# mihikamd/DP-GSAT

Hardware: AMD Instinct MI355X
Metric: million edges/s (attn+sample+aggregate fwd+bwd) (higher is better)
Workload: dtype f32

## Files before the change

dp_gsat_amd/csrc/common.h:

```cpp
#pragma once
#include <cstring>
#include <cstdint>
#include <cstdio>
#include <cstdarg>
#include <hip/hip_runtime.h>

#include "../../include/gsat_hip.h"

namespace gsat {

void set_error(const char* fmt, ...);
const char* get_error();

#define GSAT_CHECK_HIP(expr)                                                                  \
    do {                                                                                      \
        hipError_t _e = (expr);                                                               \
        if (_e != hipSuccess) {                                                               \
            gsat::set_error("%s:%d: %s -> %s", __FILE__, __LINE__, #expr, hipGetErrorString(_e)); \
            return GSAT_ERR_HIP;                                                              \
        }                                                                                     \
    } while (0)

#define GSAT_REQUIRE(cond, code, ...)                                                         \
    do {                                                                                      \
        if (!(cond)) {                                                                        \
            gsat::set_error(__VA_ARGS__);                                                     \
            return (code);                                                                    \
        }                                                                                     \
    } while (0)

#define GSAT_LAUNCH_CHECK() GSAT_CHECK_HIP(hipGetLastError())

static inline int64_t ceil_div(int64_t a, int64_t b) { return (a + b - 1) / b; }

hipError_t zero_async(void* p, size_t bytes, hipStream_t stream);
static inline size_t align_up(size_t a, size_t b) { return (a + b - 1) / b * b; }

struct Arena {
    char* base;
    size_t cap, off;
    Arena(void* p, size_t bytes) : base(static_cast<char*>(p)), cap(bytes), off(0) {}
    template <class T> T* take(size_t n) {
        size_t b = align_up(n * sizeof(T), 256);
        if (base == nullptr || off + b > cap) { off += b; return nullptr; }
        T* r = reinterpret_cast<T*>(base + off);
        off += b;
        return r;
    }
    bool ok() const { return base != nullptr && off <= cap; }
};

struct SlabJob { const float* ws; int nslab; size_t slab; int M, N; int64_t ldc; int accumulate; float* out; };
int gemm_f32(hipStream_t stream, bool a_t, bool b_t, int64_t M, int64_t N, int64_t K, const float* A, int64_t lda, const float* B,
             int64_t ldb, float* C, int64_t ldc, const float* bias, bool accumulate, float* ws, size_t ws_floats, bool allow_split = false,
             SlabJob* defer = nullptr);
int slab_reduce_jobs(hipStream_t stream, const SlabJob* jobs, int n);
size_t gemm_workspace_floats(int64_t M, int64_t N, int64_t K, bool reduce_rows);

int aggr_sum_fwd_impl(hipStream_t stream, const float* x, const float* self_rows, const float* att, const float* edge_emb,
                      const int32_t* rowptr, const int32_t* col, const int32_t* eid, int64_t N, int64_t E, int64_t H, float self_coef,
                      float* out, const int32_t* chunk_ptr, float* partial);

#ifdef __HIPCC__
constexpr int WAVE = 64;

template <int CTRL> __device__ __forceinline__ float dpp_add(float v) {
    const int t = __builtin_amdgcn_update_dpp(0, __builtin_bit_cast(int, v), CTRL, 0xF, 0xF, true);
    return v + __builtin_bit_cast(float, t);
}

template <int WIDTH> __device__ __forceinline__ float group_sum(float v) {
    if constexpr ((WIDTH & (WIDTH - 1)) == 0) {
        if constexpr (WIDTH >= 2) v = dpp_add<0xB1>(v);
        if constexpr (WIDTH >= 4) v = dpp_add<0x4E>(v);
        if constexpr (WIDTH >= 8) v = dpp_add<0x141>(v);
        if constexpr (WIDTH >= 16) v = dpp_add<0x140>(v);
        if constexpr (WIDTH >= 32) v += __builtin_bit_cast(float, __builtin_amdgcn_ds_swizzle(__builtin_bit_cast(int, v), 0x401F));
        if constexpr (WIDTH >= 64) v += __shfl_xor(v, 32, 64);
    } else {
        const int l = (int)(threadIdx.x & 63) % WIDTH;
#pragma unroll
        for (int o = 16; o > 0; o >>= 1) {
            const float t = __shfl_down(v, o, 64);
            if (l + o < WIDTH) v += t;
        }
    }
    return v;
}

template <int LPR, int BLOCK> struct LaneGroups {
    static constexpr int GPW = 64 / LPR, GPB = (BLOCK / 64) * GPW;
    int grp, lane;
    __device__ __forceinline__ LaneGroups() {
        const int wl = threadIdx.x & 63, sub = wl / LPR;
        lane = wl % LPR;
        grp = sub < GPW ? (int)(threadIdx.x >> 6) * GPW + sub : -1;
    }
};

__device__ __forceinline__ float4 ld4(const float* p) { return *reinterpret_cast<const float4*>(p); }
__device__ __forceinline__ void st4(float* p, float4 v) { *reinterpret_cast<float4*>(p) = v; }
__device__ __forceinline__ void st4_nt(float* p, float4 v) {
    typedef float v4f __attribute__((ext_vector_type(4)));
    v4f t = {v.x, v.y, v.z, v.w};
    __builtin_nontemporal_store(t, reinterpret_cast<v4f*>(p));
}
__device__ __forceinline__ float4 f4zero() { return make_float4(0.f, 0.f, 0.f, 0.f); }
__device__ __forceinline__ float4 f4fma(float a, float4 x, float4 acc) {
    acc.x = fmaf(a, x.x, acc.x); acc.y = fmaf(a, x.y, acc.y);
    acc.z = fmaf(a, x.z, acc.z); acc.w = fmaf(a, x.w, acc.w);
    return acc;
}
__device__ __forceinline__ float f4dot(float4 a, float4 b) {
    return fmaf(a.x, b.x, fmaf(a.y, b.y, fmaf(a.z, b.z, a.w * b.w)));
}

__device__ __forceinline__ uint4 philox4x32(uint64_t seed, uint32_t c0, uint32_t c1, uint32_t c2, uint32_t c3) {
    uint32_t k0 = (uint32_t)seed, k1 = (uint32_t)(seed >> 32);
#pragma unroll
    for (int r = 0; r < 10; ++r) {
        uint64_t p0 = (uint64_t)0xD2511F53u * c0;
        uint64_t p1 = (uint64_t)0xCD9E8D57u * c2;
        uint32_t n0 = (uint32_t)(p1 >> 32) ^ c1 ^ k0;
        uint32_t n1 = (uint32_t)p1;
        uint32_t n2 = (uint32_t)(p0 >> 32) ^ c3 ^ k1;
        uint32_t n3 = (uint32_t)p0;
        c0 = n0; c1 = n1; c2 = n2; c3 = n3;
        k0 += 0x9E3779B9u; k1 += 0xBB67AE85u;
    }
    return make_uint4(c0, c1, c2, c3);
}

__device__ __forceinline__ float philox_noise_u(uint64_t seed, int row) {
    const uint4 r = philox4x32(seed, (uint32_t)row, 0u, 4u, 0x5A17u);
    return ((float)(r.x >> 9) + 0.5f) * (1.0f / 8388608.0f);
}

struct SeedRef {
    uint64_t value;
    const uint64_t* dev;
    __device__ __forceinline__ uint64_t get() const { return dev ? *dev : value; }
};

__device__ __forceinline__ float4 philox_keep4(uint64_t seed, int layer, int row, int c, float p) {
    uint4 r = philox4x32(seed, (uint32_t)row, (uint32_t)(c >> 2), (uint32_t)layer, 0x5A17u);
    const float k = 1.0f / 16777216.0f;
    return make_float4((float)(r.x >> 8) * k >= p ? 1.f : 0.f, (float)(r.y >> 8) * k >= p ? 1.f : 0.f,
                       (float)(r.z >> 8) * k >= p ? 1.f : 0.f, (float)(r.w >> 8) * k >= p ? 1.f : 0.f);
}
#endif

}
```

dp_gsat_amd/csrc/pna.hip:

```cpp
#include "common.h"
#include "pna_math.h"

namespace gsat {

constexpr int PNA_BLOCK = 128;
constexpr int SC_AMP = GSAT_SCALE_AMPLIFICATION, SC_ATT = GSAT_SCALE_ATTENUATION, SC_LIN = GSAT_SCALE_LINEAR, SC_INVLIN = GSAT_SCALE_INVERSE_LINEAR;

struct PnaCfg {
    int A, S;
    int aggr[8];
    int scal[8];
    float avg_lin, avg_log;
};

__device__ __forceinline__ int pna_xcd_remap(int b, int nb) {
    int q = nb >> 3, r = nb & 7, x = b & 7, i = b >> 3;
    return (x < r ? x * (q + 1) : r * (q + 1) + (x - r) * q) + i;
}

__device__ __forceinline__ float scaler_factor(int s, float deg, float avg_lin, float avg_log) {
    switch (s) {
        case SC_AMP: return logf(deg + 1.f) / avg_log;
        case SC_ATT: return deg == 0.f ? 1.f : avg_log / logf(deg + 1.f);
        case SC_LIN: return deg / avg_lin;
// ... 473 lines not shown
                P = make_float4(p0.x - mean.x * Q.x, p0.y - mean.y * Q.y, p0.z - mean.z * Q.z, p0.w - mean.w * Q.w);   \
            }
            GSAT_FOLD(ai, 0, Pi, Qi, gmn_i, gmx_i)
            {
#define GSAT_SELF(C)                                                                                                   \
            {                                                                                                          \
                const float xc = xi.C;                                                                                 \
                const float wlo = xc > 0.f ? amin : (xc < 0.f ? amax : wfirst), whi = xc > 0.f ? amax : (xc < 0.f ? amin : wfirst); \
                dxi.C = Pi.C * sa + Qi.C * xc * sa2 + gmn_i.C * wlo + gmx_i.C * whi;                                   \
                t1 = fmaf(Pi.C, xc, t1);                                                                               \
                t2 = fmaf(Qi.C * xc, xc, t2);                                                                          \
                tmn += xc > 0.f ? gmn_i.C * xc : (xc < 0.f ? gmx_i.C * xc : 0.f);                                      \
                tmx += xc > 0.f ? gmx_i.C * xc : (xc < 0.f ? gmn_i.C * xc : 0.f);                                      \
            }
            float4 dxi;
            GSAT_SELF(x) GSAT_SELF(y) GSAT_SELF(z) GSAT_SELF(w)
#undef GSAT_SELF
            st4(dx_self + (size_t)row * H + c, dxi);
            }
            GSAT_FOLD(aj, 1, Pj, Qj, gmn_j, gmx_j)
            if (HAS_EE) { GSAT_FOLD(ae, 2, Pe, Qe, gmn_e, gmx_e) }
#undef GSAT_FOLD
        }
        if (LONG) {
            float* r = partial + (size_t)chunk_ptr[row] * rec;
            if (on) {
                st4(r + c, Pj); st4(r + H + c, Qj); st4(r + 2 * H + c, gmn_j); st4(r + 3 * H + c, gmx_j);
                st4i(r + 4 * H + c, jmin); st4i(r + 5 * H + c, jmax);
                if (HAS_EE) {
                    float* re = r + 6 * H;
                    st4(re + c, Pe); st4(re + H + c, Qe); st4(re + 2 * H + c, gmn_e); st4(re + 3 * H + c, gmx_e);
                    st4i(re + 4 * H + c, emin); st4i(re + 5 * H + c, emax);
                }
            }
            const float s1 = group_sum<LPR>(t1), s2 = group_sum<LPR>(t2), smn = group_sum<LPR>(tmn), smx = group_sum<LPR>(tmx);
            if (lane == 0) {
                st4(r + (size_t)6 * GP * H, make_float4(s1, s2, smn, smx));
                st4(r + (size_t)6 * GP * H + 4, make_float4(__int_as_float(kmin_a), __int_as_float(kmax_a), 0.f, 0.f));
            }
            continue;
        }
        for (int kb = beg; kb < end; kb += 4) {
            const int nb = min(4, end - kb);
            int j4[4], e4[4];
            float w4[4];
            float4 x4[4], ee4[4];
            if (end - beg <= 4) {
#pragma unroll
                for (int u = 0; u < 4; ++u) { j4[u] = lj[u]; e4[u] = le[u]; w4[u] = lw[u]; }
            } else {
#pragma unroll
                for (int u = 0; u < 4; ++u) {
                    j4[u] = u < nb ? col[kb + u] : 0;
                    e4[u] = u < nb ? eid[kb + u] : 0;
                }
#pragma unroll
                for (int u = 0; u < 4; ++u) w4[u] = (u < nb && att) ? att[e4[u]] : 1.f;
            }
#pragma unroll
            for (int u = 0; u < 4; ++u) {
                x4[u] = (u < nb && on) ? ld4(x + (size_t)j4[u] * H + c) : f4zero();
                if (HAS_EE) ee4[u] = (u < nb && on) ? ld4(edge_emb + (size_t)e4[u] * H + c) : f4zero();
            }
#pragma unroll
            for (int u = 0; u < 4; ++u) {
                if (u >= nb) continue;
                const int k = kb + u, e = e4[u];
                const float w = w4[u];
                const float4 xj = x4[u];
                float da = 0.f;
                if (on) {
                    float4 dm;
                    dm.x = fmaf(Qj.x, w * xj.x, Pj.x) + (k == jmin.x ? gmn_j.x : 0.f) + (k == jmax.x ? gmx_j.x : 0.f);
                    dm.y = fmaf(Qj.y, w * xj.y, Pj.y) + (k == jmin.y ? gmn_j.y : 0.f) + (k == jmax.y ? gmx_j.y : 0.f);
                    dm.z = fmaf(Qj.z, w * xj.z, Pj.z) + (k == jmin.z ? gmn_j.z : 0.f) + (k == jmax.z ? gmx_j.z : 0.f);
                    dm.w = fmaf(Qj.w, w * xj.w, Pj.w) + (k == jmin.w ? gmn_j.w : 0.f) + (k == jmax.w ? gmx_j.w : 0.f);
                    st4(dmsg + (size_t)k * H + c, f4scale(w, dm));
                    da += f4dot(dm, xj);
                    da += t1 + w * t2 + (k == kmin_a ? tmn : 0.f) + (k == kmax_a ? tmx : 0.f);
                    if (HAS_EE) {
                        const float4 ee = ee4[u];
                        float4 de;
                        de.x = fmaf(Qe.x, w * ee.x, Pe.x) + (k == emin.x ? gmn_e.x : 0.f) + (k == emax.x ? gmx_e.x : 0.f);
                        de.y = fmaf(Qe.y, w * ee.y, Pe.y) + (k == emin.y ? gmn_e.y : 0.f) + (k == emax.y ? gmx_e.y : 0.f);
                        de.z = fmaf(Qe.z, w * ee.z, Pe.z) + (k == emin.z ? gmn_e.z : 0.f) + (k == emax.z ? gmx_e.z : 0.f);
                        de.w = fmaf(Qe.w, w * ee.w, Pe.w) + (k == emin.w ? gmn_e.w : 0.f) + (k == emax.w ? gmx_e.w : 0.f);
                        if (dedge) st4(dedge + (size_t)e * H + c, f4scale(w, de));
                        da += f4dot(de, ee);
                    }
                }
                if (datt) {
                    da = group_sum<LPR>(da);
                    if (lane == 0) datt[e] = c0 ? datt[e] + da : da;
                }
            }
        }
    }
}

constexpr int TILE_BLOCK = 512;

__global__ void k_pna_tiles(const int32_t* __restrict__ node_ptr, const int32_t* __restrict__ node_seg, const int32_t* __restrict__ rowptr,
                            const int32_t* __restrict__ rowptr_src, int N, int TN, int slack, int T, int4* __restrict__ desc,
                            int32_t* __restrict__ spill_count) {
    const int t = blockIdx.x * blockDim.x + threadIdx.x;
    if (t == 0 && spill_count) *spill_count = 0;
    if (t > T) return;
    const int64_t p = (int64_t)t * TN;
    int start = N;
    if (t < T && p < N) {
        start = (int)p;
        if (node_seg) {
            const int g0 = node_ptr[node_seg[p]];
            start = min((int)p, max(g0, (int)p - slack));
        }
    }
    desc[t] = make_int4(start, rowptr[start], rowptr_src[start], 0);
}

template <int LPR, int NAGG, bool NATT>
__global__ __launch_bounds__(TILE_BLOCK, 4) void k_pna_bwd_tile(
    const float* __restrict__ x, const float* __restrict__ att, const float* __restrict__ dout, const int32_t* __restrict__ rowptr,
    const int32_t* __restrict__ col, const int32_t* __restrict__ eid, const int4* __restrict__ desc,
    const int32_t* __restrict__ rowptr_src, const int32_t* __restrict__ slot_map, int H, int TE, int RCAP, float* dx,
    float* __restrict__ dmsg, float* datt, float* __restrict__ dw, const float* __restrict__ dx_add, int datt_acc) {
    constexpr int GPB = LaneGroups<LPR, TILE_BLOCK>::GPB;
    constexpr int RPW = 64 / LPR;
    constexpr int NSEG = NAGG * 2;
    extern __shared__ float4 smem4[];
    float4* erow = smem4;
    int* s_col = reinterpret_cast<int*>(erow + (size_t)TE * LPR);
    int* s_eid = s_col + TE;
    float* s_w = reinterpret_cast<float*>(s_eid);
    float* s_att = reinterpret_cast<float*>(s_eid + TE);
    int* s_slot = reinterpret_cast<int*>(s_att + TE);
    int* s_rp = s_slot + TE;
    int* s_rps = s_rp + RCAP + 1;
    float* s_na = reinterpret_cast<float*>(s_rps + RCAP + 1);
    float* s_dna = s_na + RCAP + 1;
    const int tid = threadIdx.x, wave = tid >> 6;
    const LaneGroups<LPR, TILE_BLOCK> lg;
    const int grp = lg.grp < 0 ? GPB : lg.grp;
    const int lane = lg.lane, c = lane * 4;
    const bool on = c < H && lg.grp >= 0;
    const int t = pna_xcd_remap(blockIdx.x, gridDim.x);
    const int4 d0 = desc[t], d1 = desc[t + 1];
    const int n0 = d0.x, n1 = d1.x;
    if (n1 <= n0) return;
    const int nr = n1 - n0;
    const int k0 = d0.y, ne = min(d1.y - k0, TE);
    const int s0 = d0.z, ns = d1.z - s0, nsl = min(ns, TE);
    float4 dcur[NSEG];
    float4 xi_cur = f4zero();
    const size_t out_stride = (size_t)NSEG * H;
    int row = lg.grp >= 0 ? n0 + grp : n1;
#pragma unroll
    for (int sg = 0; sg < NSEG; ++sg) dcur[sg] = f4zero();
    if (row < n1 && on) {
        const float* g0 = dout + (size_t)row * out_stride + c;
#pragma unroll
        for (int sg = 0; sg < NSEG; ++sg) dcur[sg] = ld4(g0 + (size_t)sg * H);
        xi_cur = ld4(x + (size_t)row * H + c);
    }
    for (int i = tid; i <= nr; i += TILE_BLOCK) {
        s_rp[i] = rowptr[n0 + i] - k0;
        s_rps[i] = rowptr_src[n0 + i] - s0;
        if (NATT) { s_na[i] = att[min(n0 + i, n1 - 1)]; s_dna[i] = 0.f; }
    }
    for (int i = tid; i < ne; i += TILE_BLOCK) {
        s_col[i] = col[k0 + i];
        if (!NATT) s_eid[i] = eid[k0 + i];
    }
    for (int i = tid; i < nsl; i += TILE_BLOCK) s_slot[i] = slot_map[s0 + i] - k0;
    __syncthreads();
    for (int base = 0; base < ne; base += GPB) {
        const int i = base + grp;
        if (i < ne && on)
            __builtin_amdgcn_global_load_lds((const __attribute__((address_space(1))) void*)(x + (size_t)s_col[i] * H + c),
                                             (__attribute__((address_space(3))) void*)(erow + (size_t)(base + wave * RPW) * LPR), 16, 0, 0);
    }
    for (int i = tid; i < ne; i += TILE_BLOCK) {
        if (NATT) {
            int lo = 0, hi = nr;
            while (hi - lo > 1) { const int mid = (lo + hi) >> 1; if (s_rp[mid] <= i) lo = mid; else hi = mid; }
            const float a = att[s_col[i]];
            s_att[i] = a;
            s_w[i] = a * s_na[lo];
        } else {
            s_att[i] = att ? att[s_eid[i]] : 1.f;
        }
    }
    asm volatile("s_waitcnt vmcnt(0)" ::: "memory");
    __syncthreads();
    for (; row < n1; row += GPB) {
        const int nrow = row + GPB;
        const int beg = s_rp[row - n0], end = s_rp[row - n0 + 1];
        const float cnt = (float)(end - beg);
        float sa = 0.f, sa2 = 0.f, amin = INFINITY, amax = -INFINITY;
        int kmin_a = beg, kmax_a = beg;
        Acc4 aj;
        aj.init();
        int4 jmin = make_int4(beg, beg, beg, beg), jmax = jmin;
        float wfirst = 1.f;
        for (int k = beg; k < end; ++k) {
            float w;
            float4 xv;
            if (k < ne) {
                w = NATT ? s_w[k] : s_att[k];
                xv = on ? erow[(size_t)k * LPR + lane] : f4zero();
            } else {
                w = NATT ? att[col[k0 + k]] * s_na[row - n0] : (att ? att[eid[k0 + k]] : 1.f);
                xv = on ? ld4(x + (size_t)col[k0 + k] * H + c) : f4zero();
            }
            if (k == beg) wfirst = w;
            sa += w; sa2 = fmaf(w, w, sa2);
            if (w < amin) { amin = w; kmin_a = k; }
            if (w > amax) { amax = w; kmax_a = k; }
            const float4 m = f4scale(w, xv);
            if (m.x < aj.mn.x) jmin.x = k; if (m.y < aj.mn.y) jmin.y = k; if (m.z < aj.mn.z) jmin.z = k; if (m.w < aj.mn.w) jmin.w = k;
            if (m.x > aj.mx.x) jmax.x = k; if (m.y > aj.mx.y) jmax.y = k; if (m.z > aj.mx.z) jmax.z = k; if (m.w > aj.mx.w) jmax.w = k;
            aj.add(m);
        }
        const float4 xi = xi_cur;
        const Acc4 ai = self_stats(xi, sa, sa2, amin, amax);
        const float n = fmaxf(cnt, 1.f), inv_n = 1.f / n;
        float t1 = 0.f, t2 = 0.f, tmn = 0.f, tmx = 0.f;
        float4 Pi, Qi, Pj, Qj, gmn_i, gmx_i, gmn_j, gmx_j;
#define GSAT_TFOLD(ACC, PART, P, Q, GMN, GMX)                                                                              \
        {                                                                                                                  \
            const float4 mean = f4scale(inv_n, ACC.s);                                                                     \
            const float4 var = make_float4(ACC.q.x * inv_n - mean.x * mean.x, ACC.q.y * inv_n - mean.y * mean.y,           \
                                           ACC.q.z * inv_n - mean.z * mean.z, ACC.q.w * inv_n - mean.w * mean.w);          \
            const float4 hs = make_float4(var.x > 0.f ? 0.5f * __builtin_amdgcn_rsqf(var.x + 1e-5f) : 0.f,                 \
                                          var.y > 0.f ? 0.5f * __builtin_amdgcn_rsqf(var.y + 1e-5f) : 0.f,                 \
                                          var.z > 0.f ? 0.5f * __builtin_amdgcn_rsqf(var.z + 1e-5f) : 0.f,                 \
                                          var.w > 0.f ? 0.5f * __builtin_amdgcn_rsqf(var.w + 1e-5f) : 0.f);                \
            float4 p0 = f4scale(inv_n, dcur[0 * 2 + (PART)]);                                                              \
            if (NAGG == 5) { const float4 vsum = dcur[(NAGG == 5 ? 4 : 0) * 2 + (PART)];                                   \
                             p0 = make_float4(p0.x + vsum.x, p0.y + vsum.y, p0.z + vsum.z, p0.w + vsum.w); }               \
            GMN = dcur[1 * 2 + (PART)];                                                                                    \
            GMX = dcur[2 * 2 + (PART)];                                                                                    \
            const float4 vs = dcur[3 * 2 + (PART)];                                                                        \
            const float4 gv = make_float4(vs.x * hs.x, vs.y * hs.y, vs.z * hs.z, vs.w * hs.w);                             \
            Q = f4scale(2.f * inv_n, gv);                                                                                  \
            P = make_float4(p0.x - mean.x * Q.x, p0.y - mean.y * Q.y, p0.z - mean.z * Q.z, p0.w - mean.w * Q.w);           \
        }
        GSAT_TFOLD(ai, 0, Pi, Qi, gmn_i, gmx_i)
        GSAT_TFOLD(aj, 1, Pj, Qj, gmn_j, gmx_j)
#undef GSAT_TFOLD
        if (nrow < n1 && on) {
            const float* g0 = dout + (size_t)nrow * out_stride + c;
#pragma unroll
            for (int sg = 0; sg < NSEG; ++sg) dcur[sg] = ld4(g0 + (size_t)sg * H);
            xi_cur = ld4(x + (size_t)nrow * H + c);
        }
        if (on) {
            float4 dxi;
#define GSAT_TSELF(C)                                                                                                      \
            {                                                                                                              \
                const float xc = xi.C;                                                                                     \
                const float wlo = xc > 0.f ? amin : (xc < 0.f ? amax : wfirst), whi = xc > 0.f ? amax : (xc < 0.f ? amin : wfirst); \
                dxi.C = Pi.C * sa + Qi.C * xc * sa2 + gmn_i.C * wlo + gmx_i.C * whi;                                       \
                t1 = fmaf(Pi.C, xc, t1);                                                                                   \
                t2 = fmaf(Qi.C * xc, xc, t2);                                                                              \
                tmn += xc > 0.f ? gmn_i.C * xc : (xc < 0.f ? gmx_i.C * xc : 0.f);                                          \
                tmx += xc > 0.f ? gmx_i.C * xc : (xc < 0.f ? gmn_i.C * xc : 0.f);                                          \
            }
            GSAT_TSELF(x) GSAT_TSELF(y) GSAT_TSELF(z) GSAT_TSELF(w)
#undef GSAT_TSELF
            if (end == beg) dxi = f4zero();
            st4(dx + (size_t)row * H + c, dxi);
        }
        for (int k = beg; k < end; ++k) {
            float w;
            float4 xj;
            int e = 0, j;
            if (k < ne) {
                w = NATT ? s_w[k] : s_att[k]; j = s_col[k];
                if (!NATT) e = s_eid[k];
                xj = on ? erow[(size_t)k * LPR + lane] : f4zero();
            } else {
                j = col[k0 + k];
                if (!NATT) e = eid[k0 + k];
                w = NATT ? att[j] * s_na[row - n0] : (att ? att[e] : 1.f);
                xj = on ? ld4(x + (size_t)j * H + c) : f4zero();
            }
            const bool in_lds = k < ne && j >= n0 && j < n1;
            float da = 0.f;
            if (on) {
                float4 dm;
                dm.x = fmaf(Qj.x, w * xj.x, Pj.x) + (k == jmin.x ? gmn_j.x : 0.f) + (k == jmax.x ? gmx_j.x : 0.f);
                dm.y = fmaf(Qj.y, w * xj.y, Pj.y) + (k == jmin.y ? gmn_j.y : 0.f) + (k == jmax.y ? gmx_j.y : 0.f);
                dm.z = fmaf(Qj.z, w * xj.z, Pj.z) + (k == jmin.z ? gmn_j.z : 0.f) + (k == jmax.z ? gmx_j.z : 0.f);
                dm.w = fmaf(Qj.w, w * xj.w, Pj.w) + (k == jmin.w ? gmn_j.w : 0.f) + (k == jmax.w ? gmx_j.w : 0.f);
                const float4 o = f4scale(w, dm);
                if (in_lds) erow[(size_t)k * LPR + lane] = o; else st4(dmsg + (size_t)(k0 + k) * H + c, o);
                da = f4dot(dm, xj) + t1 + w * t2 + (k == kmin_a ? tmn : 0.f) + (k == kmax_a ? tmx : 0.f);
            }
            if (datt) {
                da = group_sum<LPR>(da);
                if (NATT) {
                    if (lane == 0) {
                        s_dna[row - n0] = fmaf(da, k < ne ? s_att[k] : att[j], s_dna[row - n0]);
                        const float share = da * s_na[row - n0];
                        if (in_lds) s_w[k] = share; else dw[k0 + k] = share;
                    }
                } else if (lane == 0) datt[e] = da;
            }
        }
    }
    __syncthreads();
    for (int j = lg.grp >= 0 ? n0 + grp : n1; j < n1; j += GPB) {
        if (!on) continue;
        const int sb = s_rps[j - n0], se = s_rps[j - n0 + 1];
        float4 acc = ld4(dx + (size_t)j * H + c);
        const float dprev = (NATT && datt && datt_acc && lane == 0) ? datt[j] : 0.f;
        if (dx_add) {
            const float4 r = ld4(dx_add + (size_t)j * H + c);
            acc.x += r.x; acc.y += r.y; acc.z += r.z; acc.w += r.w;
        }
        float sw = 0.f;
        for (int s_ = sb; s_ < se; ++s_) {
            const int kl = s_ < nsl ? s_slot[s_] : slot_map[s0 + s_] - k0;
            if (kl >= 0 && kl < ne) {
                const float4 v = erow[(size_t)kl * LPR + lane];
                acc.x += v.x; acc.y += v.y; acc.z += v.z; acc.w += v.w;
                if (NATT) sw += s_w[kl];
            }
        }
        st4(dx + (size_t)j * H + c, acc);
        if (NATT && datt && lane == 0) datt[j] = (s_dna[j - n0] + sw) + dprev;
    }
}

__global__ void k_pna_spill_rows(const int4* __restrict__ desc, int TN, int TE, const int32_t* __restrict__ rowptr_src,
                                 const int32_t* __restrict__ slot_map, int num_rows, int32_t* __restrict__ spill_rows,
                                 int32_t* __restrict__ spill_count) {
    const int j = blockIdx.x * blockDim.x + threadIdx.x;
    if (j >= num_rows) return;
    const int sb = rowptr_src[j], se = rowptr_src[j + 1];
    if (sb == se) return;
    int t = j / TN;
    if (j >= desc[t + 1].x) ++t;
    const int k0 = desc[t].y, ne = min(desc[t + 1].y - k0, TE);
    bool flag = false;
    for (int s_ = sb; s_ < se && !flag; ++s_) {
        const int k = slot_map[s_];
        flag = k < k0 || k >= k0 + ne;
    }
    if (flag) {
        const int idx = atomicAdd(spill_count, 1);
        if (idx < num_rows) spill_rows[idx] = j;
    }
}

template <int LPR>
__global__ __launch_bounds__(256) void k_pna_bwd_spill(const float* __restrict__ dmsg, const int4* __restrict__ desc, int TN, int TE,
                                                       const int32_t* __restrict__ rowptr_src, const int32_t* __restrict__ slot_map,
                                                       const int32_t* __restrict__ spill_rows, const int32_t* __restrict__ spill_count,
                                                       int num_rows, int H, float* __restrict__ dx, const float* __restrict__ dw,
                                                       float* __restrict__ dna) {
    const LaneGroups<LPR, 256> lg;
    constexpr int GPB = LaneGroups<LPR, 256>::GPB;
    const int lane = lg.lane, c = lane * 4;
    const int count = min(*spill_count, num_rows);
    if (lg.grp < 0) return;
    for (int i = blockIdx.x * GPB + lg.grp; i < count; i += gridDim.x * GPB) {
        const int j = spill_rows[i];
        const int sb = rowptr_src[j], se = rowptr_src[j + 1];
        int t = j / TN;
        if (j >= desc[t + 1].x) ++t;
        const int k0 = desc[t].y, ne = min(desc[t + 1].y - k0, TE);
        if (c >= H) continue;
        float4 acc = ld4(dx + (size_t)j * H + c);
        float sw = 0.f;
        for (int s_ = sb; s_ < se; ++s_) {
            const int k = slot_map[s_];
            if (k >= k0 && k < k0 + ne) continue;
            const float4 v = ld4(dmsg + (size_t)k * H + c);
            acc.x += v.x; acc.y += v.y; acc.z += v.z; acc.w += v.w;
            if (dna) sw += dw[k];
        }
        st4(dx + (size_t)j * H + c, acc);
        if (dna && lane == 0) dna[j] += sw;
    }
}

static inline int pna_lpr(int64_t H) {
    if (H <= 0 || H % 4 != 0 || H > 256) return 0;
    int64_t q = H / 4;
    return q <= 4 ? 4 : q <= 8 ? 8 : q <= 16 ? 16 : q <= 20 ? 20 : q <= 32 ? 32 : 64;
}

constexpr int PNA_CHUNK = 256;
static inline bool pna_width_ok(int64_t H) { return H > 0 && H % 4 == 0 && H <= 512; }

static inline void pna_grid(int64_t N, int lpr, int* nb, int* rpg) {
    const int gpb = (PNA_BLOCK / 64) * (64 / lpr);
    int64_t b = ceil_div(N, gpb);
    if (b > 256 * 64) b = 256 * 64;
    if (b < 1) b = 1;
    *nb = (int)b;
    *rpg = (int)std::max<int64_t>(1, ceil_div(N, b * gpb));
}

static inline int fixed_aggregators(const PnaCfg& cfg) {
    if (cfg.S != 1 || cfg.scal[0] != 0 || (cfg.A != 4 && cfg.A != 5)) return 0;
    if (cfg.aggr[0] != AGG_MEAN || cfg.aggr[1] != AGG_MIN || cfg.aggr[2] != AGG_MAX || cfg.aggr[3] != GSAT_AGG_STD) return 0;
    if (cfg.A == 5 && cfg.aggr[4] != AGG_SUM) return 0;
    return cfg.A;
}

static int make_cfg(const int32_t* aggr, int A, const int32_t* scal, int S, float avg_lin, float avg_log, PnaCfg* cfg) {
    GSAT_REQUIRE(aggr && scal && A >= 1 && A <= 8 && S >= 1 && S <= 8, GSAT_ERR_ARG, "pna: need 1..8 aggregators and scalers");
    cfg->A = A; cfg->S = S; cfg->avg_lin = avg_lin; cfg->avg_log = avg_log;
    for (int i = 0; i < 8; ++i) { cfg->aggr[i] = 0; cfg->scal[i] = 0; }
    for (int i = 0; i < A; ++i) {
        GSAT_REQUIRE(aggr[i] >= 0 && aggr[i] <= 5, GSAT_ERR_ARG, "pna: unknown aggregator code %d", aggr[i]);
        cfg->aggr[i] = aggr[i];
    }
    for (int i = 0; i < S; ++i) {
        GSAT_REQUIRE(scal[i] >= 0 && scal[i] <= 4, GSAT_ERR_ARG, "pna: unknown scaler code %d", scal[i]);
        cfg->scal[i] = scal[i];
    }
    return GSAT_OK;
}

template <int L, int NA, bool NATT>
static hipError_t pna_tile_allow_lds(size_t lds) {
    static size_t allowed = 0;
    if (lds <= allowed) return hipSuccess;
    hipError_t e = hipFuncSetAttribute((const void*)k_pna_bwd_tile<L, NA, NATT>, hipFuncAttributeMaxDynamicSharedMemorySize, (int)lds);
    if (e == hipSuccess) allowed = lds;
    return e;
}

static size_t pna_tile_lds_bytes(int lpr, int edges_cap, int rows_cap) {
    return (size_t)edges_cap * ((size_t)lpr * 16 + 16) + (size_t)(rows_cap + 1) * 16;
}

}

using namespace gsat;

#define GSAT_LPR_DISPATCH(lpr, CALL) \
    switch (lpr) { case 4: CALL(4); break; case 8: CALL(8); break; case 16: CALL(16); break; case 20: CALL(20); break; case 32: CALL(32); break; default: CALL(64); break; }

extern "C" {

static int pna_fwd_impl(const char* who, const float* x, const float* att, const float* edge_emb, const int32_t* rowptr, const int32_t* col,
                        const int32_t* eid, int64_t N, int64_t E, int64_t H, const int32_t* aggregators, int A, const int32_t* scalers, int S,
                        float avg_deg_lin, float avg_deg_log, float* out, const int32_t* chunk_ptr, float* partial, hipStream_t stream,
                        float* scal_out = nullptr) {
    GSAT_REQUIRE(N >= 0 && N < (1ll << 31), GSAT_ERR_ARG, "%s: bad N", who);
    PnaCfg cfg;
    int rc = make_cfg(aggregators, A, scalers, S, avg_deg_lin, avg_deg_log, &cfg);
    if (rc) return rc;
    if (N == 0) return GSAT_OK;
    GSAT_REQUIRE(pna_width_ok(H), GSAT_ERR_UNSUPPORTED, "%s: H=%lld must be a multiple of 4 and <= 512", who, (long long)H);
    GSAT_REQUIRE(x && rowptr && out, GSAT_ERR_ARG, "%s: null pointer", who);
    GSAT_REQUIRE(chunk_ptr == nullptr || partial != nullptr, GSAT_ERR_ARG, "%s: chunk_ptr needs the record workspace", who);
    if (E <= CH) chunk_ptr = nullptr;
    const int nagg = fixed_aggregators(cfg);
    GSAT_REQUIRE(!scal_out || (nagg && !edge_emb && !chunk_ptr), GSAT_ERR_UNSUPPORTED,
                 "%s: the compact output needs (mean,min,max,std[,sum]) with the identity scaler, no edge features, no hub chunks", who);
    for (int c0 = 0; c0 < (int)H; c0 += PNA_CHUNK) {
        const int Hc = std::min<int>(PNA_CHUNK, (int)H - c0);
        const int lpr = pna_lpr(Hc);
        int nb, rpg;
        pna_grid(N, lpr, &nb, &rpg);
        const int gpb = (PNA_BLOCK / 64) * (64 / lpr);
        const int cb = chunk_ptr ? (int)std::min<int64_t>(ceil_div(pna_max_chunks(E), gpb), 256 * 16) : 0;
#define GO(L, EE, NA)                                                                                                                       \
    do {                                                                                                                                    \
        k_pna_fwd<L, EE, NA, false><<<nb, PNA_BLOCK, 0, stream>>>(x, att, edge_emb, rowptr, col, eid, (int)N, (int)H, cfg, out, rpg, c0, Hc, chunk_ptr, partial, scal_out); \
        if (cb) k_pna_fwd<L, EE, NA, true><<<cb, PNA_BLOCK, 0, stream>>>(x, att, edge_emb, rowptr, col, eid, (int)N, (int)H, cfg, out, rpg, c0, Hc, chunk_ptr, partial, scal_out); \
    } while (0)
#define CALL(L)                                                                                                              \
    do {                                                                                                                     \
        if (edge_emb) {                                                                                                      \
            if (cb) k_pna_chunk_stats<L, true><<<cb, PNA_BLOCK, 0, stream>>>(x, att, edge_emb, rowptr, col, eid, (int)N, (int)H, chunk_ptr, partial, c0, Hc); \
            if (nagg == 4) GO(L, true, 4); else if (nagg == 5) GO(L, true, 5); else GO(L, true, 0);                          \
        } else {                                                                                                             \
            if (cb) k_pna_chunk_stats<L, false><<<cb, PNA_BLOCK, 0, stream>>>(x, att, edge_emb, rowptr, col, eid, (int)N, (int)H, chunk_ptr, partial, c0, Hc); \
// ... 213 lines not shown
```

Measured before the change: 125.4.

## Streamline PNA tiled backward: window-relative 32-bit addressing, split LDS/global edge loops

Rewrites the tiled PNA backward kernel to address global data through per-tile base pointers with 32-bit byte offsets. It splits each row's edge loop into an LDS-resident part and a global part so the inner loops no longer branch per edge. The per-edge binary search that built s_w at tile setup is removed, and the weight is computed as att*na_row inline. Each row's d-node-attention is accumulated in a register, explicit LDS store intrinsics are used, and the last row's dx is kept in a register instead of being re-read from global memory. The aim is fewer address computations, branches and memory round-trips, at the cost of more code and a risk of 32-bit offset overflow on large tiles.

```diff
diff --git a/dp_gsat_amd/csrc/common.h b/dp_gsat_amd/csrc/common.h
--- a/dp_gsat_amd/csrc/common.h
+++ b/dp_gsat_amd/csrc/common.h
@@ -105,6 +105,18 @@
     v4f t = {v.x, v.y, v.z, v.w};
     __builtin_nontemporal_store(t, reinterpret_cast<v4f*>(p));
 }
+__device__ __forceinline__ float4 ld4_off(const float* base, uint32_t byte_off) {
+    return *reinterpret_cast<const float4*>(reinterpret_cast<const char*>(base) + byte_off);
+}
+__device__ __forceinline__ void st4_off(float* base, uint32_t byte_off, float4 v) {
+    *reinterpret_cast<float4*>(reinterpret_cast<char*>(base) + byte_off) = v;
+}
+__device__ __forceinline__ void st4_lds(float4* p, float4 v) {
+    typedef float v4f __attribute__((ext_vector_type(4)));
+    v4f t = {v.x, v.y, v.z, v.w};
+    *(__attribute__((address_space(3))) v4f*)p = t;
+}
+__device__ __forceinline__ void st1_lds(float* p, float v) { *(__attribute__((address_space(3))) float*)p = v; }
 __device__ __forceinline__ float4 f4zero() { return make_float4(0.f, 0.f, 0.f, 0.f); }
 __device__ __forceinline__ float4 f4fma(float a, float4 x, float4 acc) {
     acc.x = fmaf(a, x.x, acc.x); acc.y = fmaf(a, x.y, acc.y);
diff --git a/dp_gsat_amd/csrc/pna.hip b/dp_gsat_amd/csrc/pna.hip
--- a/dp_gsat_amd/csrc/pna.hip
+++ b/dp_gsat_amd/csrc/pna.hip
@@ -649,15 +649,18 @@
     const int s0 = d0.z, ns = d1.z - s0, nsl = min(ns, TE);
     float4 dcur[NSEG];
     float4 xi_cur = f4zero();
-    const size_t out_stride = (size_t)NSEG * H;
-    int row = lg.grp >= 0 ? n0 + grp : n1;
+    const uint32_t hb = (uint32_t)H * 4u, gb = NSEG * hb, cb = (uint32_t)c * 4u;
+    const float* gwin = dout + (size_t)n0 * NSEG * H;
+    const float* xwin = x + (size_t)n0 * H;
+    float* dxwin = dx + (size_t)n0 * H;
+    float* mwin = dmsg + (size_t)k0 * H;
+    int r = lg.grp >= 0 ? grp : nr;
 #pragma unroll
     for (int sg = 0; sg < NSEG; ++sg) dcur[sg] = f4zero();
-    if (row < n1 && on) {
-        const float* g0 = dout + (size_t)row * out_stride + c;
-#pragma unroll
-        for (int sg = 0; sg < NSEG; ++sg) dcur[sg] = ld4(g0 + (size_t)sg * H);
-        xi_cur = ld4(x + (size_t)row * H + c);
+    if (r < nr && on) {
+#pragma unroll
+        for (int sg = 0; sg < NSEG; ++sg) dcur[sg] = ld4_off(gwin, r * gb + sg * hb + cb);
+        xi_cur = ld4_off(xwin, r * hb + cb);
     }
     for (int i = tid; i <= nr; i += TILE_BLOCK) {
         s_rp[i] = rowptr[n0 + i] - k0;
@@ -678,20 +681,18 @@
     }
     for (int i = tid; i < ne; i += TILE_BLOCK) {
         if (NATT) {
-            int lo = 0, hi = nr;
-            while (hi - lo > 1) { const int mid = (lo + hi) >> 1; if (s_rp[mid] <= i) lo = mid; else hi = mid; }
-            const float a = att[s_col[i]];
-            s_att[i] = a;
-            s_w[i] = a * s_na[lo];
+            s_att[i] = att[s_col[i]];
         } else {
             s_att[i] = att ? att[s_eid[i]] : 1.f;
         }
     }
     asm volatile("s_waitcnt vmcnt(0)" ::: "memory");
     __syncthreads();
-    for (; row < n1; row += GPB) {
-        const int nrow = row + GPB;
-        const int beg = s_rp[row - n0], end = s_rp[row - n0 + 1];
+    float4 dx_keep = f4zero();
+    for (; r < nr; r += GPB) {
+        const int nr_ = r + GPB;
+        const int beg = s_rp[r], end = s_rp[r + 1];
+        const float na_row = NATT ? s_na[r] : 0.f;
         const float cnt = (float)(end - beg);
         float sa = 0.f, sa2 = 0.f, amin = INFINITY, amax = -INFINITY;
         int kmin_a = beg, kmax_a = beg;
@@ -699,25 +700,25 @@
         aj.init();
         int4 jmin = make_int4(beg, beg, beg, beg), jmax = jmin;
         float wfirst = 1.f;
-        for (int k = beg; k < end; ++k) {
-            float w;
-            float4 xv;
-            if (k < ne) {
-                w = NATT ? s_w[k] : s_att[k];
-                xv = on ? erow[(size_t)k * LPR + lane] : f4zero();
-            } else {
-                w = NATT ? att[col[k0 + k]] * s_na[row - n0] : (att ? att[eid[k0 + k]] : 1.f);
-                xv = on ? ld4(x + (size_t)col[k0 + k] * H + c) : f4zero();
-            }
+        const int mid = min(end, max(beg, ne));
+        auto stats = [&](int k, float w, float4 xv) {
             if (k == beg) wfirst = w;
             sa += w; sa2 = fmaf(w, w, sa2);
             if (w < amin) { amin = w; kmin_a = k; }
             if (w > amax) { amax = w; kmax_a = k; }
             const float4 m = f4scale(w, xv);
-            if (m.x < aj.mn.x) jmin.x = k; if (m.y < aj.mn.y) jmin.y = k; if (m.z < aj.mn.z) jmin.z = k; if (m.w < aj.mn.w) jmin.w = k;
-            if (m.x > aj.mx.x) jmax.x = k; if (m.y > aj.mx.y) jmax.y = k; if (m.z > aj.mx.z) jmax.z = k; if (m.w > aj.mx.w) jmax.w = k;
-            aj.add(m);
-        }
+#define GSAT_TARG(C)                                                                                                       \
+            if (m.C < aj.mn.C) { jmin.C = k; aj.mn.C = m.C; }                                                              \
+            if (m.C > aj.mx.C) { jmax.C = k; aj.mx.C = m.C; }
+            GSAT_TARG(x) GSAT_TARG(y) GSAT_TARG(z) GSAT_TARG(w)
+#undef GSAT_TARG
+            aj.s.x += m.x; aj.s.y += m.y; aj.s.z += m.z; aj.s.w += m.w;
+            aj.q.x = fmaf(m.x, m.x, aj.q.x); aj.q.y = fmaf(m.y, m.y, aj.q.y); aj.q.z = fmaf(m.z, m.z, aj.q.z); aj.q.w = fmaf(m.w, m.w, aj.q.w);
+        };
+        for (int k = beg; k < mid; ++k)
+            stats(k, NATT ? s_att[k] * na_row : s_att[k], on ? erow[(size_t)k * LPR + lane] : f4zero());
+        for (int k = mid; k < end; ++k)
+            stats(k, NATT ? att[col[k0 + k]] * na_row : (att ? att[eid[k0 + k]] : 1.f), on ? ld4(x + (size_t)col[k0 + k] * H + c) : f4zero());
         const float4 xi = xi_cur;
         const Acc4 ai = self_stats(xi, sa, sa2, amin, amax);
         const float n = fmaxf(cnt, 1.f), inv_n = 1.f / n;
@@ -743,14 +744,6 @@
             P = make_float4(p0.x - mean.x * Q.x, p0.y - mean.y * Q.y, p0.z - mean.z * Q.z, p0.w - mean.w * Q.w);           \
         }
         GSAT_TFOLD(ai, 0, Pi, Qi, gmn_i, gmx_i)
-        GSAT_TFOLD(aj, 1, Pj, Qj, gmn_j, gmx_j)
-#undef GSAT_TFOLD
-        if (nrow < n1 && on) {
-            const float* g0 = dout + (size_t)nrow * out_stride + c;
-#pragma unroll
-            for (int sg = 0; sg < NSEG; ++sg) dcur[sg] = ld4(g0 + (size_t)sg * H);
-            xi_cur = ld4(x + (size_t)nrow * H + c);
-        }
         if (on) {
             float4 dxi;
 #define GSAT_TSELF(C)                                                                                                      \
@@ -766,23 +759,18 @@
             GSAT_TSELF(x) GSAT_TSELF(y) GSAT_TSELF(z) GSAT_TSELF(w)
 #undef GSAT_TSELF
             if (end == beg) dxi = f4zero();
-            st4(dx + (size_t)row * H + c, dxi);
-        }
-        for (int k = beg; k < end; ++k) {
-            float w;
-            float4 xj;
-            int e = 0, j;
-            if (k < ne) {
-                w = NATT ? s_w[k] : s_att[k]; j = s_col[k];
-                if (!NATT) e = s_eid[k];
-                xj = on ? erow[(size_t)k * LPR + lane] : f4zero();
-            } else {
-                j = col[k0 + k];
-                if (!NATT) e = eid[k0 + k];
-                w = NATT ? att[j] * s_na[row - n0] : (att ? att[e] : 1.f);
-                xj = on ? ld4(x + (size_t)j * H + c) : f4zero();
-            }
-            const bool in_lds = k < ne && j >= n0 && j < n1;
+            if (nr_ < nr) st4_off(dxwin, r * hb + cb, dxi); else dx_keep = dxi;
+        }
+        GSAT_TFOLD(aj, 1, Pj, Qj, gmn_j, gmx_j)
+#undef GSAT_TFOLD
+        if (nr_ < nr && on) {
+#pragma unroll
+            for (int sg = 0; sg < NSEG; ++sg) dcur[sg] = ld4_off(gwin, nr_ * gb + sg * hb + cb);
+            xi_cur = ld4_off(xwin, nr_ * hb + cb);
+        }
+        float dna_acc = 0.f;
+        auto grad = [&](int k, float w, float a_src, int j, int e, float4 xj, bool lds) {
+            const bool in_lds = lds && j >= n0 && j < n1;
             float da = 0.f;
             if (on) {
                 float4 dm;
@@ -791,30 +779,43 @@
                 dm.z = fmaf(Qj.z, w * xj.z, Pj.z) + (k == jmin.z ? gmn_j.z : 0.f) + (k == jmax.z ? gmx_j.z : 0.f);
                 dm.w = fmaf(Qj.w, w * xj.w, Pj.w) + (k == jmin.w ? gmn_j.w : 0.f) + (k == jmax.w ? gmx_j.w : 0.f);
                 const float4 o = f4scale(w, dm);
-                if (in_lds) erow[(size_t)k * LPR + lane] = o; else st4(dmsg + (size_t)(k0 + k) * H + c, o);
+                if (in_lds) st4_lds(erow + (size_t)k * LPR + lane, o);
+                else if (lds) st4_off(mwin, k * hb + cb, o);
+                else st4(dmsg + (size_t)(k0 + k) * H + c, o);
                 da = f4dot(dm, xj) + t1 + w * t2 + (k == kmin_a ? tmn : 0.f) + (k == kmax_a ? tmx : 0.f);
             }
             if (datt) {
                 da = group_sum<LPR>(da);
                 if (NATT) {
                     if (lane == 0) {
-                        s_dna[row - n0] = fmaf(da, k < ne ? s_att[k] : att[j], s_dna[row - n0]);
-                        const float share = da * s_na[row - n0];
-                        if (in_lds) s_w[k] = share; else dw[k0 + k] = share;
+                        dna_acc = fmaf(da, a_src, dna_acc);
+                        const float share = da * na_row;
+                        if (in_lds) st1_lds(s_w + k, share); else dw[k0 + k] = share;
                     }
                 } else if (lane == 0) datt[e] = da;
             }
-        }
+        };
+        for (int k = beg; k < mid; ++k) {
+            const float a = s_att[k];
+            grad(k, NATT ? a * na_row : a, a, s_col[k], NATT ? 0 : s_eid[k], on ? erow[(size_t)k * LPR + lane] : f4zero(), true);
+        }
+        for (int k = mid; k < end; ++k) {
+            const int j = col[k0 + k], e = NATT ? 0 : eid[k0 + k];
+            const float a = NATT ? att[j] : (att ? att[e] : 1.f);
+            grad(k, NATT ? a * na_row : a, a, j, e, on ? ld4(x + (size_t)j * H + c) : f4zero(), false);
+        }
+        if (NATT && datt && lane == 0) s_dna[r] = dna_acc;
     }
     __syncthreads();
-    for (int j = lg.grp >= 0 ? n0 + grp : n1; j < n1; j += GPB) {
+    const float* awin = dx_add ? dx_add + (size_t)n0 * H : nullptr;
+    for (int j = lg.grp >= 0 ? grp : nr; j < nr; j += GPB) {
         if (!on) continue;
-        const int sb = s_rps[j - n0], se = s_rps[j - n0 + 1];
-        float4 acc = ld4(dx + (size_t)j * H + c);
-        const float dprev = (NATT && datt && datt_acc && lane == 0) ? datt[j] : 0.f;
-        if (dx_add) {
-            const float4 r = ld4(dx_add + (size_t)j * H + c);
-            acc.x += r.x; acc.y += r.y; acc.z += r.z; acc.w += r.w;
+        const int sb = s_rps[j], se = s_rps[j + 1];
+        float4 acc = j + GPB < nr ? ld4_off(dxwin, j * hb + cb) : dx_keep;
+        const float dprev = (NATT && datt && datt_acc && lane == 0) ? datt[n0 + j] : 0.f;
+        if (awin) {
+            const float4 ra = ld4_off(awin, j * hb + cb);
+            acc.x += ra.x; acc.y += ra.y; acc.z += ra.z; acc.w += ra.w;
         }
         float sw = 0.f;
         for (int s_ = sb; s_ < se; ++s_) {
@@ -822,11 +823,11 @@
             if (kl >= 0 && kl < ne) {
                 const float4 v = erow[(size_t)kl * LPR + lane];
                 acc.x += v.x; acc.y += v.y; acc.z += v.z; acc.w += v.w;
-                if (NATT) sw += s_w[kl];
-            }
-        }
-        st4(dx + (size_t)j * H + c, acc);
-        if (NATT && datt && lane == 0) datt[j] = (s_dna[j - n0] + sw) + dprev;
+                if (NATT && datt) sw += s_w[kl];
+            }
+        }
+        st4_off(dxwin, j * hb + cb, acc);
+        if (NATT && datt && lane == 0) datt[n0 + j] = (s_dna[j] + sw) + dprev;
     }
 }
 
```

Result: faster. 129.4, median of 6 (+3.2%).
